# EdwinZhanCN/Lumen

Measured on AMD Instinct MI355X. Metric: CLIP ViT-L/14 images/sec (whole node), higher is better.
Workload: dtype bf16; 1 GPU; model=CLIP ViT-L-14 image tower, global_batch=512, seq_len=257, parallelism=dp1, image_size=224, per_gpu_batch=512

## Files before the change

lumen_amd/csrc/attention.hip:

```cpp
#include <cstdlib>
#include <type_traits>
#include "attention.h"
#include "common.h"
#include "tuning.h"

namespace lumen {

typedef short s16x4v __attribute__((ext_vector_type(4)));

template <int D>
__device__ __forceinline__ int k_phys(int row, int chunk) {
  if constexpr (D == 64) return chunk ^ ((row >> 1) & 7);
  else if constexpr (D == 128) return chunk ^ (row & 15);
  else return chunk ^ ((row >> 2) & 3);
}
template <int D>
__device__ __forceinline__ int v_phys(int row, int chunk) {
  if constexpr (D == 64) return chunk ^ (((row >> 1) & 3) << 1);
  else if constexpr (D == 128) return chunk ^ ((row & 7) << 1);
  else return chunk ^ (((row >> 2) & 1) << 1);
}

__device__ __forceinline__ float vmax_raw(float a, float b) {
  float r;
  asm("v_max_f32_e32 %0, %1, %2" : "=v"(r) : "v"(a), "v"(b));
  return r;
}
__device__ __forceinline__ float group4_max(float x) {
  const auto r = __builtin_amdgcn_permlane16_swap(__float_as_uint(x), __float_as_uint(x), false, false);
  x = vmax_raw(__uint_as_float(r[0]), __uint_as_float(r[1]));
  const auto s = __builtin_amdgcn_permlane32_swap(__float_as_uint(x), __float_as_uint(x), false, false);
  return vmax_raw(__uint_as_float(s[0]), __uint_as_float(s[1]));
}

__device__ __forceinline__ s16x4v ds_read_tr16(const char* p) {
  typedef __attribute__((address_space(3))) s16x4v* lp;
  return __builtin_amdgcn_ds_read_tr16_b64_v4i16((lp)(p));
}
typedef __attribute__((address_space(3))) const char lds_char;
__device__ __forceinline__ s16x4v ds_read_tr16(const lds_char* p) {
  typedef __attribute__((address_space(3))) s16x4v* lp;
  return __builtin_amdgcn_ds_read_tr16_b64_v4i16((lp)(p));
}

template <int NB, int MASK>
__device__ __forceinline__ void softmax_chunk(f32x4_t (&sc)[4], f32x4_t (&o)[NB], f32x4_t& l4, float& mrow,
                                              const AttnArgs& a, bool need_mask, int k0, int g, int qi,
                                              int kv_len, int causal_off) {
  float mx = -INFINITY;
  if (MASK == 1 || (MASK == 2 && need_mask)) {
#pragma unroll
    for (int kb16 = 0; kb16 < 4; ++kb16)
#pragma unroll
      for (int r = 0; r < 4; ++r) {
        const int kj = k0 + kb16 * 16 + g * 4 + r;
        bool ok = kj < kv_len;
        if (a.causal) ok = ok && (kj <= qi + causal_off);
        const float sv = ok ? sc[kb16][r] : -INFINITY;
        sc[kb16][r] = sv;
        mx = fmaxf(mx, sv);
      }
  } else {
#pragma unroll
    for (int kb16 = 0; kb16 < 4; ++kb16)
#pragma unroll
      for (int r = 0; r < 4; ++r) mx = fmaxf(mx, sc[kb16][r]);
  }
  mx = group4_max(mx);
  const float mcand = vmax_raw(mrow, mx * a.scale_log2);
  if (__any(mcand > mrow + 8.f)) {
    const float mb = mcand == -INFINITY ? 0.f : mcand;
    const float alpha = __builtin_amdgcn_exp2f(mrow - mb);
#pragma unroll
    for (int j = 0; j < NB; ++j) o[j] *= alpha;
    l4 *= alpha;
    mrow = mcand;
  }
  const float nmb = mrow == -INFINITY ? 0.f : -mrow;
#pragma unroll
  for (int kb16 = 0; kb16 < 4; ++kb16)
#pragma unroll
    for (int r = 0; r < 4; ++r) sc[kb16][r] = __builtin_amdgcn_exp2f(__builtin_fmaf(sc[kb16][r], a.scale_log2, nmb));
}

__device__ __forceinline__ bf16x8_t ones_bf16x8() {
  return __builtin_bit_cast(bf16x8_t, (s16x8_t){0x3F80, 0x3F80, 0x3F80, 0x3F80, 0x3F80, 0x3F80, 0x3F80, 0x3F80});
}

template <int D, int NW = 4>
__global__ void __launch_bounds__(64 * NW) attn_fwd_kernel(AttnArgs a) {
  constexpr int NCH = D / 8;
  constexpr int KS = D / 32;
  constexpr int NB = D / 16;
  constexpr int KC = 64;
  constexpr int IMG = KC * D * 2;
  constexpr int RPI = 1024 / (D * 2);
  constexpr int NI = KC / RPI / NW;
  constexpr int QB = 16 * NW;
  static_assert(NI >= 1, "K/V staging");
  __shared__ __attribute__((aligned(16))) char smem[2 * 2 * IMG];

  const int tid = threadIdx.x, lane = tid & 63;
  const int wid = __builtin_amdgcn_readfirstlane(tid >> 6);
  const int col = lane & 15, g = lane >> 4;
  const int nqb = gridDim.x;
  const int lin = xcd_remap(blockIdx.x + nqb * (blockIdx.y + gridDim.y * blockIdx.z), nqb * gridDim.y * gridDim.z);
  const int qblk = a.causal ? nqb - 1 - lin % nqb : lin % nqb;
  const int h = (lin / nqb) % gridDim.y, b = lin / (nqb * gridDim.y);
  const int hk = h / (a.H / a.Hkv);
  const int q0 = qblk * QB + wid * 16;
  const int kv_len = a.kv_len ? min(a.kv_len[b], a.Sk) : a.Sk;
  const int causal_off = a.Sk - a.Sq;

  const uint16_t* qb = a.q + b * a.q_sb + h * a.q_sh;
  const uint16_t* kb = a.k + b * a.k_sb + hk * a.k_sh;
  const uint16_t* vb = a.v + b * a.v_sb + hk * a.v_sh;

  bf16x8_t qf[KS];
  {
    const int qr = min(q0 + col, a.Sq - 1);
#pragma unroll
    for (int t = 0; t < KS; ++t) qf[t] = *(const bf16x8_t*)(qb + (int64_t)qr * a.q_ss + t * 32 + g * 8);
  }

  typedef __attribute__((address_space(3))) void* lds_ptr_t;
  typedef const __attribute__((address_space(1))) void* g_ptr_t;
  int srow[NI], kch[NI], vch[NI];
#pragma unroll
  for (int i = 0; i < NI; ++i) {
    const int r = (wid * NI + i) * RPI + lane / NCH;
    const int pc = lane % NCH;
    srow[i] = r;
    kch[i] = k_phys<D>(r, pc);
    vch[i] = v_phys<D>(r, pc);
  }
  auto stage = [&](int chunk, int buf) {
    const int k0 = chunk * KC;
#pragma unroll
    for (int i = 0; i < NI; ++i) {
      const int kr = min(k0 + srow[i], a.Sk - 1);
      char* dk = smem + buf * 2 * IMG + (wid * NI + i) * 1024;
      __builtin_amdgcn_global_load_lds((g_ptr_t)(kb + (int64_t)kr * a.k_ss + kch[i] * 8), (lds_ptr_t)dk, 16, 0, 0);
      __builtin_amdgcn_global_load_lds((g_ptr_t)(vb + (int64_t)kr * a.v_ss + vch[i] * 8), (lds_ptr_t)(dk + IMG), 16,
                                       0, 0);
    }
  };

  f32x4_t o[NB];
#pragma unroll
  for (int j = 0; j < NB; ++j) o[j] = (f32x4_t){0.f, 0.f, 0.f, 0.f};
  float mrow = -INFINITY;
  f32x4_t l4 = (f32x4_t){0.f, 0.f, 0.f, 0.f};
  const int qi = q0 + col;

  int kend = kv_len;
  if (a.causal) kend = min(kend, min(qblk * QB + QB, a.Sq) + causal_off);
  const int nkc = (kend + KC - 1) / KC;

  const bool active = q0 < a.Sq;
  const int wave_kend = a.causal ? min(kend, min(q0 + 16, a.Sq) + causal_off) : kend;

  if (nkc > 0) stage(0, 0);
  for (int kc = 0; kc < nkc; ++kc) {
    const int buf = kc & 1;
    asm volatile("s_waitcnt vmcnt(0)" ::: "memory");
    __syncthreads();
    if (kc + 1 < nkc) stage(kc + 1, buf ^ 1);
    const int k0 = kc * KC;
    if (!active || k0 >= wave_kend) continue;
    const char* sK = smem + buf * 2 * IMG;
    const char* sV = sK + IMG;

    f32x4_t sc[4];
#pragma unroll
    for (int kb16 = 0; kb16 < 4; ++kb16) {
      sc[kb16] = (f32x4_t){0.f, 0.f, 0.f, 0.f};
      const int kr = kb16 * 16 + col;
#pragma unroll
      for (int t = 0; t < KS; ++t) {
        bf16x8_t kf = *(const bf16x8_t*)(sK + kr * D * 2 + (k_phys<D>(kr, t * 4 + g) << 4));
        sc[kb16] = __builtin_amdgcn_mfma_f32_16x16x32_bf16(kf, qf[t], sc[kb16], 0, 0, 0);
      }
    }
    const bool need_mask = (k0 + KC > kv_len) || (a.causal && k0 + KC - 1 > q0 + causal_off);
    softmax_chunk<NB, 2>(sc, o, l4, mrow, a, need_mask, k0, g, qi, kv_len, causal_off);

#pragma unroll
    for (int s = 0; s < 2; ++s) {
      bf16x8_t pf;
#pragma unroll
      for (int r = 0; r < 4; ++r) {
        pf[r] = (__bf16)sc[2 * s][r];
        pf[4 + r] = (__bf16)sc[2 * s + 1][r];
      }
      const int q = col >> 2, p = col & 3;
      const int r0 = s * 32 + 4 * g + q, r1 = r0 + 16;
#pragma unroll
      for (int j = 0; j < NB; ++j) {
        const int c0 = j * 16 + 4 * p;
        const char* a0 = sV + r0 * D * 2 + (v_phys<D>(r0, c0 >> 3) << 4) + (c0 & 7) * 2;
        const char* a1 = sV + r1 * D * 2 + (v_phys<D>(r1, c0 >> 3) << 4) + (c0 & 7) * 2;
        const s16x4v lo = ds_read_tr16(a0);
        const s16x4v hi = ds_read_tr16(a1);
        s16x8_t vv = (s16x8_t){lo[0], lo[1], lo[2], lo[3], hi[0], hi[1], hi[2], hi[3]};
        o[j] = __builtin_amdgcn_mfma_f32_16x16x32_bf16(__builtin_bit_cast(bf16x8_t, vv), pf, o[j], 0, 0, 0);
      }
      l4 = __builtin_amdgcn_mfma_f32_16x16x32_bf16(ones_bf16x8(), pf, l4, 0, 0, 0);
    }
  }

  const float inv = l4[0] > 0.f ? __builtin_amdgcn_rcpf(l4[0]) : 0.f;
  if (a.o != nullptr && qi < a.Sq) {
    uint16_t* orow = a.o + b * a.o_sb + h * a.o_sh + (int64_t)qi * a.o_ss;
#pragma unroll
    for (int j = 0; j < NB; ++j) {
      uint2 w;
      w.x = pack2bf(o[j][0] * inv, o[j][1] * inv);
      w.y = pack2bf(o[j][2] * inv, o[j][3] * inv);
      *(uint2*)(orow + j * 16 + 4 * g) = w;
    }
  }
  if constexpr (D >= 64) {
    if (a.o8 != nullptr) {
      constexpr int NM = D / 32;
      float am[NM];
#pragma unroll
      for (int m = 0; m < NM; ++m) {
        float x = 0.f;
#pragma unroll
        for (int r = 0; r < 4; ++r) x = fmaxf(x, fmaxf(fabsf(o[2 * m][r]), fabsf(o[2 * m + 1][r])));
        x *= inv;
        x = fmaxf(x, __shfl_xor(x, 16, 64));
        am[m] = fmaxf(x, __shfl_xor(x, 32, 64));
      }
      if (qi < a.Sq) {
        uint8_t* o8 = a.o8 + b * a.o8_sb + (int64_t)qi * a.o8_ss + h * D;
        uint32_t sbytes = 0;
#pragma unroll
        for (int m = 0; m < NM; ++m) {
          const int e = mx_exp(am[m]);
          const float sc = inv * mx_inv(e);
          sbytes |= (uint32_t)(e + 127) << (8 * m);
#pragma unroll
          for (int jj = 0; jj < 2; ++jj) {
            const int j = 2 * m + jj;
            float t[4];
#pragma unroll
            for (int r = 0; r < 4; ++r) t[r] = fminf(fmaxf(o[j][r] * sc, -448.f), 448.f);
            int w = __builtin_amdgcn_cvt_pk_fp8_f32(t[0], t[1], 0, false);
            w = __builtin_amdgcn_cvt_pk_fp8_f32(t[2], t[3], w, true);
            *(uint32_t*)(o8 + j * 16 + 4 * g) = (uint32_t)w;
          }
        }
        uint8_t* os = a.os + b * a.os_sb + (int64_t)((h * D) >> 7) * a.os_ss + (int64_t)qi * 4 + ((h * NM) & 3);
        if (g == 0) {
          if constexpr (NM == 4) *(uint32_t*)os = sbytes;
          else *(uint16_t*)os = (uint16_t)sbytes;
        }
      }
    }
  }
}

template <int D, int NW>
__global__ void __launch_bounds__(64 * NW) attn_res_kernel(AttnArgs a, int nkc, int clean_split) {
  constexpr int NCH = D / 8;
  constexpr int KS = D / 32;
  constexpr int NB = D / 16;
  constexpr int KC = 64;
  constexpr int IMG = KC * D * 2;
  constexpr int RPI = 1024 / (D * 2);
  constexpr int NI = KC / RPI / NW;
  static_assert(NI >= 1, "K/V staging: at least one 1 KiB DMA piece per wave per chunk");
  extern __shared__ __attribute__((aligned(16))) char smem[];

  const int tid = threadIdx.x, lane = tid & 63;
  const int wid = __builtin_amdgcn_readfirstlane(tid >> 6);
  const int col = lane & 15, g = lane >> 4;
  const int lin = xcd_remap(blockIdx.x + gridDim.x * blockIdx.y, gridDim.x * gridDim.y);
  const int h = lin % a.H, b = lin / a.H;
  const int hk = h / (a.H / a.Hkv);
  const int kv_len = a.kv_len ? min(a.kv_len[b], a.Sk) : a.Sk;
  const int causal_off = a.Sk - a.Sq;
  const uint16_t* qb = a.q + b * a.q_sb + h * a.q_sh;
  const uint16_t* kb = a.k + b * a.k_sb + hk * a.k_sh;
  const uint16_t* vb = a.v + b * a.v_sb + hk * a.v_sh;
  const __amdgpu_buffer_rsrc_t o_rs = __builtin_amdgcn_make_buffer_rsrc(
      a.o + b * a.o_sb + h * a.o_sh, (short)0, (int)(((int64_t)(a.Sq - 1) * a.o_ss + D) * 2), 0x00020000);

  const int nq16 = (a.Sq + 15) / 16;
  bf16x8_t qn[KS];
  auto load_q = [&](int blk) {
    const int qr = min(blk * 16 + col, a.Sq - 1);
#pragma unroll
    for (int t = 0; t < KS; ++t) qn[t] = *(const bf16x8_t*)(qb + (int64_t)qr * a.q_ss + t * 32 + g * 8);
  };
  load_q(wid);
  typedef __attribute__((address_space(3))) void* lds_ptr_t;
  typedef const __attribute__((address_space(1))) void* g_ptr_t;
  for (int c = 0; c < nkc; ++c) {
#pragma unroll
    for (int i = 0; i < NI; ++i) {
      const int r = (wid * NI + i) * RPI + lane / NCH;
      const int pc = lane % NCH;
      const int kr = min(c * KC + r, a.Sk - 1);
      char* dk = smem + c * 2 * IMG + (wid * NI + i) * 1024;
      __builtin_amdgcn_global_load_lds((g_ptr_t)(kb + (int64_t)kr * a.k_ss + k_phys<D>(r, pc) * 8), (lds_ptr_t)dk, 16,
                                       0, 0);
      __builtin_amdgcn_global_load_lds((g_ptr_t)(vb + (int64_t)kr * a.v_ss + v_phys<D>(r, pc) * 8),
                                       (lds_ptr_t)(dk + IMG), 16, 0, 0);
    }
  }
  asm volatile("s_waitcnt vmcnt(0)" ::: "memory");
  __syncthreads();

  int lds0 = (int)(size_t)(const lds_char*)smem;
  asm volatile("" : "+s"(lds0));
  int kofs[KS], vofs[NB];
#pragma unroll
  for (int t = 0; t < KS; ++t) kofs[t] = col * D * 2 + (k_phys<D>(col, t * 4 + g) << 4);
#pragma unroll
  for (int j = 0; j < NB; ++j) {
    const int r0 = 4 * g + (col >> 2), c0 = j * 16 + 4 * (col & 3);
    vofs[j] = r0 * D * 2 + (v_phys<D>(r0, c0 >> 3) << 4) + (c0 & 7) * 2;
  }
  auto full_chunk = [&](auto maskc, int kc, const bf16x8_t (&qf)[KS], f32x4_t (&o)[NB], f32x4_t& l4, float& mrow,
                        int q0, int qi) __attribute__((always_inline)) {
    const int k0 = kc * KC;
    const int cb = lds0 + kc * 2 * IMG;
    const lds_char* sK = (const lds_char*)(size_t)cb;
    const lds_char* sV = sK + IMG;
    f32x4_t sc[4];
#pragma unroll
    for (int kb16 = 0; kb16 < 4; ++kb16) {
      sc[kb16] = (f32x4_t){0.f, 0.f, 0.f, 0.f};
#pragma unroll
      for (int t = 0; t < KS; ++t) {
        bf16x8_t kf = *(const __attribute__((address_space(3))) bf16x8_t*)(sK + kofs[t] + kb16 * 16 * D * 2);
        sc[kb16] = __builtin_amdgcn_mfma_f32_16x16x32_bf16(kf, qf[t], sc[kb16], 0, 0, 0);
      }
    }
    softmax_chunk<NB, decltype(maskc)::value ? 1 : 0>(sc, o, l4, mrow, a, true, k0, g, qi, kv_len, causal_off);
#pragma unroll
    for (int s = 0; s < 2; ++s) {
      bf16x8_t pf;
#pragma unroll
      for (int r = 0; r < 4; ++r) {
        pf[r] = (__bf16)sc[2 * s][r];
        pf[4 + r] = (__bf16)sc[2 * s + 1][r];
      }
#pragma unroll
      for (int j = 0; j < NB; ++j) {
        const s16x4v lo = ds_read_tr16(sV + vofs[j] + s * 32 * D * 2);
        const s16x4v hi = ds_read_tr16(sV + vofs[j] + (s * 32 + 16) * D * 2);
        s16x8_t vv = (s16x8_t){lo[0], lo[1], lo[2], lo[3], hi[0], hi[1], hi[2], hi[3]};
        o[j] = __builtin_amdgcn_mfma_f32_16x16x32_bf16(__builtin_bit_cast(bf16x8_t, vv), pf, o[j], 0, 0, 0);
      }
      l4 = __builtin_amdgcn_mfma_f32_16x16x32_bf16(ones_bf16x8(), pf, l4, 0, 0, 0);
    }
  };
  auto tail_chunk = [&](int kc, const bf16x8_t (&qf)[KS], f32x4_t (&o)[NB], f32x4_t& l4, float& mrow,
                        int qi) __attribute__((always_inline)) {
    const int k0 = kc * KC;
    const char* sK = smem + kc * 2 * IMG;
    const char* sV = sK + IMG;
    f32x4_t s0 = (f32x4_t){0.f, 0.f, 0.f, 0.f};
#pragma unroll
    for (int t = 0; t < KS; ++t) {
      bf16x8_t kf = *(const bf16x8_t*)(sK + col * D * 2 + (k_phys<D>(col, t * 4 + g) << 4));
      s0 = __builtin_amdgcn_mfma_f32_16x16x32_bf16(kf, qf[t], s0, 0, 0, 0);
    }
    float mx = -INFINITY;
#pragma unroll
    for (int r = 0; r < 4; ++r) {
      const int kj = k0 + g * 4 + r;
      bool ok = kj < kv_len;
      if (a.causal) ok = ok && (kj <= qi + causal_off);
      s0[r] = ok ? s0[r] : -INFINITY;
      mx = fmaxf(mx, s0[r]);
    }
    mx = group4_max(mx);
    const float mcand = fmaxf(mrow, mx * a.scale_log2);
    if (__any(mcand > mrow + 8.f)) {
      const float mb = mcand == -INFINITY ? 0.f : mcand;
      const float alpha = __builtin_amdgcn_exp2f(mrow - mb);
#pragma unroll
      for (int j = 0; j < NB; ++j) o[j] *= alpha;
      l4 *= alpha;
      mrow = mcand;
    }
    const float nmb = mrow == -INFINITY ? 0.f : -mrow;
    bf16x8_t pf;
#pragma unroll
    for (int r = 0; r < 4; ++r) {
      pf[r] = (__bf16)__builtin_amdgcn_exp2f(__builtin_fmaf(s0[r], a.scale_log2, nmb));
      pf[4 + r] = (__bf16)0.f;
    }
    const int q = col >> 2, p = col & 3;
    const int r0 = 4 * g + q, r1 = r0 + 16;
#pragma unroll
    for (int j = 0; j < NB; ++j) {
      const int c0 = j * 16 + 4 * p;
      const char* a0 = sV + r0 * D * 2 + (v_phys<D>(r0, c0 >> 3) << 4) + (c0 & 7) * 2;
      const char* a1 = sV + r1 * D * 2 + (v_phys<D>(r1, c0 >> 3) << 4) + (c0 & 7) * 2;
      const s16x4v lo = ds_read_tr16(a0);
      const s16x4v hi = ds_read_tr16(a1);
      s16x8_t vv = (s16x8_t){lo[0], lo[1], lo[2], lo[3], hi[0], hi[1], hi[2], hi[3]};
      o[j] = __builtin_amdgcn_mfma_f32_16x16x32_bf16(__builtin_bit_cast(bf16x8_t, vv), pf, o[j], 0, 0, 0);
    }
    l4 = __builtin_amdgcn_mfma_f32_16x16x32_bf16(ones_bf16x8(), pf, l4, 0, 0, 0);
  };
  auto store_o = [&](const f32x4_t (&o)[NB], float lsum, int qi) __attribute__((always_inline)) {
    const float inv = lsum > 0.f ? __builtin_amdgcn_rcpf(lsum) : 0.f;
    const int row_off = qi * (int)a.o_ss * 2;
#pragma unroll
    for (int j = 0; j < NB; ++j) {
      typedef unsigned int u32x2v __attribute__((ext_vector_type(2)));
      const u32x2v w = {pack2bf(o[j][0] * inv, o[j][1] * inv), pack2bf(o[j][2] * inv, o[j][3] * inv)};
      __builtin_amdgcn_raw_buffer_store_b64(w, o_rs, row_off + (j * 16 + 4 * g) * 2, 0, 0);
    }
  };

  for (int qbk = wid; qbk < nq16; qbk += NW) {
    const int q0 = qbk * 16;
    const int qi = q0 + col;
    bf16x8_t qf[KS];
#pragma unroll
    for (int t = 0; t < KS; ++t) qf[t] = qn[t];
    if (qbk + NW < nq16) load_q(qbk + NW);
    f32x4_t o[NB];
#pragma unroll
    for (int j = 0; j < NB; ++j) o[j] = (f32x4_t){0.f, 0.f, 0.f, 0.f};
    float mrow = -INFINITY;
    f32x4_t l4 = (f32x4_t){0.f, 0.f, 0.f, 0.f};
    const int wave_kend = a.causal ? min(kv_len, min(q0 + 16, a.Sq) + causal_off) : kv_len;
    const int nc = min(nkc, (wave_kend + KC - 1) / KC);
    const bool tail1 = nc > 0 && wave_kend - (nc - 1) * KC <= 16;
    const int nfull = tail1 ? nc - 1 : nc;
    int nclean = clean_split ? nfull : 0;
    while (nclean > 0 && ((nclean * KC > kv_len) || (a.causal && nclean * KC - 1 > q0 + causal_off))) --nclean;
    for (int kc = 0; kc < nclean; ++kc) full_chunk(std::false_type{}, kc, qf, o, l4, mrow, q0, qi);
    for (int kc = nclean; kc < nfull; ++kc) full_chunk(std::true_type{}, kc, qf, o, l4, mrow, q0, qi);
    if (tail1) tail_chunk(nfull, qf, o, l4, mrow, qi);
    store_o(o, l4[0], qi);
  }
}

template <int D, int NW>
static hipError_t launch_res_nw(const AttnArgs& a, int B, int nkc, hipStream_t stream) {
  const size_t lds = (size_t)nkc * 2 * 64 * D * 2;
  static bool attr = false;
  if (!attr) {
    hipFuncSetAttribute((const void*)attn_res_kernel<D, NW>, hipFuncAttributeMaxDynamicSharedMemorySize, 80 * 1024);
    attr = true;
  }
  hipLaunchKernelGGL((attn_res_kernel<D, NW>), dim3(a.H, B), dim3(64 * NW), lds, stream, a, nkc,
                     tuning(TUNE_ATTN_CLEAN_CHUNKS));
  return hipGetLastError();
}

template <int D>
static hipError_t launch_res(const AttnArgs& a, int B, int nkc, hipStream_t stream) {
  const int nw = (a.Sq + 15) / 16 >= 10 ? 8 : 4;
  if constexpr (D >= 64) {
    if (nw == 8) return launch_res_nw<D, 8>(a, B, nkc, stream);
  }
  return launch_res_nw<D, 4>(a, B, nkc, stream);
}

hipError_t attn_fwd(const AttnArgs& a, int B, int D, hipStream_t stream) {
  const int nkc = (a.Sk + 63) / 64;
  if (a.o8 != nullptr && D < 64) return hipErrorInvalidValue;
  if (a.o == nullptr && a.o8 == nullptr) return hipErrorInvalidValue;
  const bool res_ok = a.o8 == nullptr && (int64_t)B * a.H >= 1024 && (size_t)nkc * 2 * 64 * D * 2 <= 80 * 1024 &&
                      a.Sq <= 1024;
  if (res_ok) {
    if (D == 64) return launch_res<64>(a, B, nkc, stream);
    if (D == 128) return launch_res<128>(a, B, nkc, stream);
    if (D == 32) return launch_res<32>(a, B, nkc, stream);
  }
  dim3 grid((a.Sq + 63) / 64, a.H, B), block(256);
  if (D == 64) hipLaunchKernelGGL((attn_fwd_kernel<64, 4>), grid, block, 0, stream, a);
  else if (D == 128) hipLaunchKernelGGL((attn_fwd_kernel<128, 4>), grid, block, 0, stream, a);
  else if (D == 32) hipLaunchKernelGGL((attn_fwd_kernel<32, 4>), grid, block, 0, stream, a);
  else return hipErrorInvalidValue;
  return hipGetLastError();
}

}
```

Measured before the change: 6531 images/s.

## Specialize resident attention kernel on causal flag and trim per-chunk overhead

Makes causal a template parameter so the non-causal path drops mask checks and uses a precomputed tail bias. It also skips the rescale on the first chunk by zero-initializing the MFMA accumulators, and precomputes 32-bit K/V/Q address offsets so address math is hoisted out of the loops. Output row offsets and the tail chunk reuse the precomputed LDS offsets. The change adds a guard on stride size for the 32-bit offsets and a second kernel instantiation.

```diff
diff --git a/lumen_amd/csrc/attention.hip b/lumen_amd/csrc/attention.hip
--- a/lumen_amd/csrc/attention.hip
+++ b/lumen_amd/csrc/attention.hip
@@ -43,7 +43,7 @@
   return __builtin_amdgcn_ds_read_tr16_b64_v4i16((lp)(p));
 }
 
-template <int NB, int MASK>
+template <int NB, int MASK, bool FIRST = false>
 __device__ __forceinline__ void softmax_chunk(f32x4_t (&sc)[4], f32x4_t (&o)[NB], f32x4_t& l4, float& mrow,
                                               const AttnArgs& a, bool need_mask, int k0, int g, int qi,
                                               int kv_len, int causal_off) {
@@ -67,14 +67,18 @@
       for (int r = 0; r < 4; ++r) mx = fmaxf(mx, sc[kb16][r]);
   }
   mx = group4_max(mx);
-  const float mcand = vmax_raw(mrow, mx * a.scale_log2);
-  if (__any(mcand > mrow + 8.f)) {
-    const float mb = mcand == -INFINITY ? 0.f : mcand;
-    const float alpha = __builtin_amdgcn_exp2f(mrow - mb);
-#pragma unroll
-    for (int j = 0; j < NB; ++j) o[j] *= alpha;
-    l4 *= alpha;
-    mrow = mcand;
+  if constexpr (FIRST) {
+    mrow = mx * a.scale_log2;
+  } else {
+    const float mcand = vmax_raw(mrow, mx * a.scale_log2);
+    if (__any(mcand > mrow + 8.f)) {
+      const float mb = mcand == -INFINITY ? 0.f : mcand;
+      const float alpha = __builtin_amdgcn_exp2f(mrow - mb);
+#pragma unroll
+      for (int j = 0; j < NB; ++j) o[j] *= alpha;
+      l4 *= alpha;
+      mrow = mcand;
+    }
   }
   const float nmb = mrow == -INFINITY ? 0.f : -mrow;
 #pragma unroll
@@ -262,7 +266,7 @@
   }
 }
 
-template <int D, int NW>
+template <int D, int NW, bool CAUSAL>
 __global__ void __launch_bounds__(64 * NW) attn_res_kernel(AttnArgs a, int nkc, int clean_split) {
   constexpr int NCH = D / 8;
   constexpr int KS = D / 32;
@@ -289,27 +293,46 @@
       a.o + b * a.o_sb + h * a.o_sh, (short)0, (int)(((int64_t)(a.Sq - 1) * a.o_ss + D) * 2), 0x00020000);
 
   const int nq16 = (a.Sq + 15) / 16;
-  bf16x8_t qn[KS];
+  bf16x8_t qn[KS] = {};
+  const uint32_t qo = (uint32_t)col * (uint32_t)a.q_ss * 2 + g * 16;
+  const uint32_t qol = (uint32_t)min(col, a.Sq - 1 - (nq16 - 1) * 16) * (uint32_t)a.q_ss * 2 + g * 16;
   auto load_q = [&](int blk) {
-    const int qr = min(blk * 16 + col, a.Sq - 1);
-#pragma unroll
-    for (int t = 0; t < KS; ++t) qn[t] = *(const bf16x8_t*)(qb + (int64_t)qr * a.q_ss + t * 32 + g * 8);
+    const char* qrow = (const char*)(qb + (int64_t)blk * 16 * a.q_ss) + (blk == nq16 - 1 ? qol : qo);
+#pragma unroll
+    for (int t = 0; t < KS; ++t) qn[t] = *(const bf16x8_t*)(qrow + t * 64);
   };
-  load_q(wid);
+  if (wid < nq16) load_q(wid);
   typedef __attribute__((address_space(3))) void* lds_ptr_t;
   typedef const __attribute__((address_space(1))) void* g_ptr_t;
-  for (int c = 0; c < nkc; ++c) {
+  if (nkc > 0) {
+    const int last_row = a.Sk - 1 - (nkc - 1) * KC;
+    uint32_t ko[NI], vo[NI], kol[NI], vol[NI];
 #pragma unroll
     for (int i = 0; i < NI; ++i) {
       const int r = (wid * NI + i) * RPI + lane / NCH;
       const int pc = lane % NCH;
-      const int kr = min(c * KC + r, a.Sk - 1);
-      char* dk = smem + c * 2 * IMG + (wid * NI + i) * 1024;
-      __builtin_amdgcn_global_load_lds((g_ptr_t)(kb + (int64_t)kr * a.k_ss + k_phys<D>(r, pc) * 8), (lds_ptr_t)dk, 16,
-                                       0, 0);
-      __builtin_amdgcn_global_load_lds((g_ptr_t)(vb + (int64_t)kr * a.v_ss + v_phys<D>(r, pc) * 8),
-                                       (lds_ptr_t)(dk + IMG), 16, 0, 0);
-    }
+      const int rl = min(r, last_row);
+      ko[i] = (uint32_t)r * (uint32_t)a.k_ss * 2 + k_phys<D>(r, pc) * 16;
+      vo[i] = (uint32_t)r * (uint32_t)a.v_ss * 2 + v_phys<D>(r, pc) * 16;
+      kol[i] = (uint32_t)rl * (uint32_t)a.k_ss * 2 + k_phys<D>(r, pc) * 16;
+      vol[i] = (uint32_t)rl * (uint32_t)a.v_ss * 2 + v_phys<D>(r, pc) * 16;
+    }
+    const char* kc_base = (const char*)kb;
+    const char* vc_base = (const char*)vb;
+    auto stage = [&](int c, const uint32_t (&kof)[NI], const uint32_t (&vof)[NI]) __attribute__((always_inline)) {
+#pragma unroll
+      for (int i = 0; i < NI; ++i) {
+        char* dk = smem + c * 2 * IMG + (wid * NI + i) * 1024;
+        __builtin_amdgcn_global_load_lds((g_ptr_t)(kc_base + kof[i]), (lds_ptr_t)dk, 16, 0, 0);
+        __builtin_amdgcn_global_load_lds((g_ptr_t)(vc_base + vof[i]), (lds_ptr_t)(dk + IMG), 16, 0, 0);
+      }
+    };
+    for (int c = 0; c < nkc - 1; ++c) {
+      stage(c, ko, vo);
+      kc_base += a.k_ss * (KC * 2);
+      vc_base += a.v_ss * (KC * 2);
+    }
+    stage(nkc - 1, kol, vol);
   }
   asm volatile("s_waitcnt vmcnt(0)" ::: "memory");
   __syncthreads();
@@ -324,8 +347,10 @@
     const int r0 = 4 * g + (col >> 2), c0 = j * 16 + 4 * (col & 3);
     vofs[j] = r0 * D * 2 + (v_phys<D>(r0, c0 >> 3) << 4) + (c0 & 7) * 2;
   }
-  auto full_chunk = [&](auto maskc, int kc, const bf16x8_t (&qf)[KS], f32x4_t (&o)[NB], f32x4_t& l4, float& mrow,
-                        int q0, int qi) __attribute__((always_inline)) {
+  auto full_chunk = [&](auto maskc, auto firstc, int kc, const bf16x8_t (&qf)[KS], f32x4_t (&o)[NB], f32x4_t& l4,
+                        float& mrow, int qi) __attribute__((always_inline)) {
+    constexpr bool FIRST = decltype(firstc)::value;
+    const f32x4_t zero4 = (f32x4_t){0.f, 0.f, 0.f, 0.f};
     const int k0 = kc * KC;
     const int cb = lds0 + kc * 2 * IMG;
     const lds_char* sK = (const lds_char*)(size_t)cb;
@@ -340,9 +365,10 @@
         sc[kb16] = __builtin_amdgcn_mfma_f32_16x16x32_bf16(kf, qf[t], sc[kb16], 0, 0, 0);
       }
     }
-    softmax_chunk<NB, decltype(maskc)::value ? 1 : 0>(sc, o, l4, mrow, a, true, k0, g, qi, kv_len, causal_off);
+    softmax_chunk<NB, decltype(maskc)::value ? 1 : 0, FIRST>(sc, o, l4, mrow, a, true, k0, g, qi, kv_len, causal_off);
 #pragma unroll
     for (int s = 0; s < 2; ++s) {
+      const bool zc = FIRST && s == 0;
       bf16x8_t pf;
 #pragma unroll
       for (int r = 0; r < 4; ++r) {
@@ -354,29 +380,31 @@
         const s16x4v lo = ds_read_tr16(sV + vofs[j] + s * 32 * D * 2);
         const s16x4v hi = ds_read_tr16(sV + vofs[j] + (s * 32 + 16) * D * 2);
         s16x8_t vv = (s16x8_t){lo[0], lo[1], lo[2], lo[3], hi[0], hi[1], hi[2], hi[3]};
-        o[j] = __builtin_amdgcn_mfma_f32_16x16x32_bf16(__builtin_bit_cast(bf16x8_t, vv), pf, o[j], 0, 0, 0);
-      }
-      l4 = __builtin_amdgcn_mfma_f32_16x16x32_bf16(ones_bf16x8(), pf, l4, 0, 0, 0);
+        o[j] = __builtin_amdgcn_mfma_f32_16x16x32_bf16(__builtin_bit_cast(bf16x8_t, vv), pf, zc ? zero4 : o[j], 0, 0,
+                                                       0);
+      }
+      l4 = __builtin_amdgcn_mfma_f32_16x16x32_bf16(ones_bf16x8(), pf, zc ? zero4 : l4, 0, 0, 0);
     }
   };
-  auto tail_chunk = [&](int kc, const bf16x8_t (&qf)[KS], f32x4_t (&o)[NB], f32x4_t& l4, float& mrow,
-                        int qi) __attribute__((always_inline)) {
+  auto tail_chunk = [&](int kc, const f32x4_t& bias, const bf16x8_t (&qf)[KS], f32x4_t (&o)[NB], f32x4_t& l4,
+                        float& mrow, int qi) __attribute__((always_inline)) {
     const int k0 = kc * KC;
-    const char* sK = smem + kc * 2 * IMG;
-    const char* sV = sK + IMG;
-    f32x4_t s0 = (f32x4_t){0.f, 0.f, 0.f, 0.f};
+    const lds_char* sK = (const lds_char*)(size_t)(lds0 + kc * 2 * IMG);
+    const lds_char* sV = sK + IMG;
+    f32x4_t s0 = bias;
 #pragma unroll
     for (int t = 0; t < KS; ++t) {
-      bf16x8_t kf = *(const bf16x8_t*)(sK + col * D * 2 + (k_phys<D>(col, t * 4 + g) << 4));
+      bf16x8_t kf = *(const __attribute__((address_space(3))) bf16x8_t*)(sK + kofs[t]);
       s0 = __builtin_amdgcn_mfma_f32_16x16x32_bf16(kf, qf[t], s0, 0, 0, 0);
     }
     float mx = -INFINITY;
 #pragma unroll
     for (int r = 0; r < 4; ++r) {
-      const int kj = k0 + g * 4 + r;
-      bool ok = kj < kv_len;
-      if (a.causal) ok = ok && (kj <= qi + causal_off);
-      s0[r] = ok ? s0[r] : -INFINITY;
+      if constexpr (CAUSAL) {
+        const int kj = k0 + g * 4 + r;
+        const bool ok = kj < kv_len && kj <= qi + causal_off;
+        s0[r] = ok ? s0[r] : -INFINITY;
+      }
       mx = fmaxf(mx, s0[r]);
     }
     mx = group4_max(mx);
@@ -396,67 +424,91 @@
       pf[r] = (__bf16)__builtin_amdgcn_exp2f(__builtin_fmaf(s0[r], a.scale_log2, nmb));
       pf[4 + r] = (__bf16)0.f;
     }
-    const int q = col >> 2, p = col & 3;
-    const int r0 = 4 * g + q, r1 = r0 + 16;
 #pragma unroll
     for (int j = 0; j < NB; ++j) {
-      const int c0 = j * 16 + 4 * p;
-      const char* a0 = sV + r0 * D * 2 + (v_phys<D>(r0, c0 >> 3) << 4) + (c0 & 7) * 2;
-      const char* a1 = sV + r1 * D * 2 + (v_phys<D>(r1, c0 >> 3) << 4) + (c0 & 7) * 2;
-      const s16x4v lo = ds_read_tr16(a0);
-      const s16x4v hi = ds_read_tr16(a1);
+      const s16x4v lo = ds_read_tr16(sV + vofs[j]);
+      const s16x4v hi = ds_read_tr16(sV + vofs[j] + 16 * D * 2);
       s16x8_t vv = (s16x8_t){lo[0], lo[1], lo[2], lo[3], hi[0], hi[1], hi[2], hi[3]};
       o[j] = __builtin_amdgcn_mfma_f32_16x16x32_bf16(__builtin_bit_cast(bf16x8_t, vv), pf, o[j], 0, 0, 0);
     }
     l4 = __builtin_amdgcn_mfma_f32_16x16x32_bf16(ones_bf16x8(), pf, l4, 0, 0, 0);
   };
-  auto store_o = [&](const f32x4_t (&o)[NB], float lsum, int qi) __attribute__((always_inline)) {
+  auto store_o = [&](const f32x4_t (&o)[NB], float lsum, int row_off) __attribute__((always_inline)) {
+    typedef float f32x2v __attribute__((ext_vector_type(2)));
+    typedef __bf16 bf16x2v __attribute__((ext_vector_type(2)));
+    typedef unsigned int u32x2v __attribute__((ext_vector_type(2)));
     const float inv = lsum > 0.f ? __builtin_amdgcn_rcpf(lsum) : 0.f;
-    const int row_off = qi * (int)a.o_ss * 2;
 #pragma unroll
     for (int j = 0; j < NB; ++j) {
-      typedef unsigned int u32x2v __attribute__((ext_vector_type(2)));
-      const u32x2v w = {pack2bf(o[j][0] * inv, o[j][1] * inv), pack2bf(o[j][2] * inv, o[j][3] * inv)};
-      __builtin_amdgcn_raw_buffer_store_b64(w, o_rs, row_off + (j * 16 + 4 * g) * 2, 0, 0);
+      const f32x2v lo = {o[j][0] * inv, o[j][1] * inv}, hi = {o[j][2] * inv, o[j][3] * inv};
+      const u32x2v w = {__builtin_bit_cast(unsigned int, __builtin_convertvector(lo, bf16x2v)),
+                        __builtin_bit_cast(unsigned int, __builtin_convertvector(hi, bf16x2v))};
+      __builtin_amdgcn_raw_buffer_store_b64(w, o_rs, row_off + j * 32, 0, 0);
     }
   };
 
-  for (int qbk = wid; qbk < nq16; qbk += NW) {
+  int nclean = 0, nfull = 0;
+  bool tail1 = false;
+  auto plan = [&](int q0) __attribute__((always_inline)) {
+    const int wave_kend = CAUSAL ? min(kv_len, min(q0 + 16, a.Sq) + causal_off) : kv_len;
+    const int nc = min(nkc, (wave_kend + KC - 1) / KC);
+    tail1 = nc > 0 && wave_kend - (nc - 1) * KC <= 16;
+    nfull = tail1 ? nc - 1 : nc;
+    nclean = min(nfull, kv_len / KC);
+    if constexpr (CAUSAL) nclean = min(nclean, max(q0 + causal_off + 1, 0) / KC);
+    if (!clean_split) nclean = 0;
+  };
+  f32x4_t tbias = (f32x4_t){0.f, 0.f, 0.f, 0.f};
+  if constexpr (!CAUSAL) {
+    plan(0);
+#pragma unroll
+    for (int r = 0; r < 4; ++r) tbias[r] = nfull * KC + g * 4 + r < kv_len ? 0.f : -INFINITY;
+  }
+
+  int row_off = ((wid * 16 + col) * (int)a.o_ss + 4 * g) * 2;
+  const int row_step = NW * 16 * (int)a.o_ss * 2;
+  for (int qbk = wid; qbk < nq16; qbk += NW, row_off += row_step) {
     const int q0 = qbk * 16;
     const int qi = q0 + col;
     bf16x8_t qf[KS];
 #pragma unroll
     for (int t = 0; t < KS; ++t) qf[t] = qn[t];
     if (qbk + NW < nq16) load_q(qbk + NW);
+    if constexpr (CAUSAL) plan(q0);
     f32x4_t o[NB];
 #pragma unroll
     for (int j = 0; j < NB; ++j) o[j] = (f32x4_t){0.f, 0.f, 0.f, 0.f};
     float mrow = -INFINITY;
     f32x4_t l4 = (f32x4_t){0.f, 0.f, 0.f, 0.f};
-    const int wave_kend = a.causal ? min(kv_len, min(q0 + 16, a.Sq) + causal_off) : kv_len;
-    const int nc = min(nkc, (wave_kend + KC - 1) / KC);
-    const bool tail1 = nc > 0 && wave_kend - (nc - 1) * KC <= 16;
-    const int nfull = tail1 ? nc - 1 : nc;
-    int nclean = clean_split ? nfull : 0;
-    while (nclean > 0 && ((nclean * KC > kv_len) || (a.causal && nclean * KC - 1 > q0 + causal_off))) --nclean;
-    for (int kc = 0; kc < nclean; ++kc) full_chunk(std::false_type{}, kc, qf, o, l4, mrow, q0, qi);
-    for (int kc = nclean; kc < nfull; ++kc) full_chunk(std::true_type{}, kc, qf, o, l4, mrow, q0, qi);
-    if (tail1) tail_chunk(nfull, qf, o, l4, mrow, qi);
-    store_o(o, l4[0], qi);
-  }
-}
-
-template <int D, int NW>
-static hipError_t launch_res_nw(const AttnArgs& a, int B, int nkc, hipStream_t stream) {
+    int kc = 0;
+    if (nclean > 0) {
+      full_chunk(std::false_type{}, std::true_type{}, 0, qf, o, l4, mrow, qi);
+      kc = 1;
+    }
+    for (; kc < nclean; ++kc) full_chunk(std::false_type{}, std::false_type{}, kc, qf, o, l4, mrow, qi);
+    for (; kc < nfull; ++kc) full_chunk(std::true_type{}, std::false_type{}, kc, qf, o, l4, mrow, qi);
+    if (tail1) tail_chunk(nfull, tbias, qf, o, l4, mrow, qi);
+    store_o(o, l4[0], row_off);
+  }
+}
+
+template <int D, int NW, bool CAUSAL>
+static hipError_t launch_res_c(const AttnArgs& a, int B, int nkc, hipStream_t stream) {
   const size_t lds = (size_t)nkc * 2 * 64 * D * 2;
   static bool attr = false;
   if (!attr) {
-    hipFuncSetAttribute((const void*)attn_res_kernel<D, NW>, hipFuncAttributeMaxDynamicSharedMemorySize, 80 * 1024);
+    (void)hipFuncSetAttribute((const void*)attn_res_kernel<D, NW, CAUSAL>, hipFuncAttributeMaxDynamicSharedMemorySize,
+                              80 * 1024);
     attr = true;
   }
-  hipLaunchKernelGGL((attn_res_kernel<D, NW>), dim3(a.H, B), dim3(64 * NW), lds, stream, a, nkc,
+  hipLaunchKernelGGL((attn_res_kernel<D, NW, CAUSAL>), dim3(a.H, B), dim3(64 * NW), lds, stream, a, nkc,
                      tuning(TUNE_ATTN_CLEAN_CHUNKS));
   return hipGetLastError();
+}
+
+template <int D, int NW>
+static hipError_t launch_res_nw(const AttnArgs& a, int B, int nkc, hipStream_t stream) {
+  return a.causal ? launch_res_c<D, NW, true>(a, B, nkc, stream) : launch_res_c<D, NW, false>(a, B, nkc, stream);
 }
 
 template <int D>
@@ -473,7 +525,8 @@
   if (a.o8 != nullptr && D < 64) return hipErrorInvalidValue;
   if (a.o == nullptr && a.o8 == nullptr) return hipErrorInvalidValue;
   const bool res_ok = a.o8 == nullptr && (int64_t)B * a.H >= 1024 && (size_t)nkc * 2 * 64 * D * 2 <= 80 * 1024 &&
-                      a.Sq <= 1024;
+                      a.Sq <= 1024 &&
+                      a.q_ss < (1 << 24) && a.k_ss < (1 << 24) && a.v_ss < (1 << 24);
   if (res_ok) {
     if (D == 64) return launch_res<64>(a, B, nkc, stream);
     if (D == 128) return launch_res<128>(a, B, nkc, stream);
```

Result: no change. 6571 images/s (median of 6 runs) (+0.6%).
